# chaitjo/efficient-gnns

Measured on NVIDIA H100. Metric: edges aggregated/s (fwd+bwd), 3-layer GCN student + logit-KD, ARXIV-shape, higher is better.
Workload: dtype f32

## Files before the change

efficient-gnns_b200/csrc/gemm_wgrad_tf32x3.cu:

```cuda
#include "common.cuh"
#include "tc_common.cuh"

namespace b200gnn {
namespace wgrad {
using namespace tc;

constexpr int BKN = 32;
constexpr int TM = 128, TN = 128;
constexpr int THREADS = 384;
constexpr int STAGES = 5;
constexpr int X_BOX = 8;
constexpr int RAW_BYTES = BKN * (TM + TN) * 4;
constexpr int OP_BYTES = 128 * BKN * 4;
constexpr int T_BYTES = 2 * OP_BYTES;
constexpr int SS_BYTES = TM / 2 * 16;
constexpr int SMEM_BYTES = STAGES * RAW_BYTES + 2 * T_BYTES + 256 + SS_BYTES + 1024;
constexpr int MAX_RANGES = 132;
constexpr int64_t MAX_PARTIAL_FLOATS = (int64_t)MAX_RANGES * 256 * 256;
constexpr int MAX_KIN = 2048, MAX_NOUT = 512;
static_assert(SMEM_BYTES <= 232448, "shared memory");

struct Params {
  float* partial;
  int32_t Nn, Kin, Kpad, Nout, Npad, num_kb;
  int32_t n_tn, n_ranges;
  const float* act_scale;
  const float* act_shift;
  const uint32_t* act_bits;
  int32_t act_words;
  float inv_keep;
  const float* act_slope;
  int32_t act_ld;
};

template <bool ACT, bool PRELU = false>
__global__ void __launch_bounds__(THREADS, 1)
wgrad_tf32x3_kernel(const __grid_constant__ CUtensorMap tmX, const __grid_constant__ CUtensorMap tmG, const Params p) {
  extern __shared__ uint8_t smem_raw[];
  uint8_t* smem = reinterpret_cast<uint8_t*>((reinterpret_cast<uintptr_t>(smem_raw) + 1023) & ~(uintptr_t)1023);
  uint8_t* tbuf = smem + STAGES * RAW_BYTES;
  uint64_t* full = reinterpret_cast<uint64_t*>(tbuf + 2 * T_BYTES);
  uint64_t* empty = full + STAGES;
  float4* act_ss = reinterpret_cast<float4*>(tbuf + 2 * T_BYTES + 256);

  const int tiles = (p.Kpad / TM) * p.n_tn;
  const int tile = (int)blockIdx.x % tiles, range = (int)blockIdx.x / tiles;
  const int mt = tile / p.n_tn, nt = tile % p.n_tn;
  const int kb0 = (int)((int64_t)p.num_kb * range / p.n_ranges);
  const int kb1 = (int)((int64_t)p.num_kb * (range + 1) / p.n_ranges);

  const int warp = threadIdx.x >> 5, lane = threadIdx.x & 31;
  if (threadIdx.x == 0) {
    for (int s = 0; s < STAGES; ++s) { mbar_init(&full[s], 1); mbar_init(&empty[s], 256); }
    asm volatile("fence.mbarrier_init.release.cluster;" ::: "memory");
  }
  __syncthreads();

  if (warp < 4) {
    regs_dec<40>();
    if (threadIdx.x == 0) {
      int s = 0; uint32_t ph = 0;
      for (int kb = kb0; kb < kb1; ++kb) {
        mbar_wait(&empty[s], ph ^ 1);
        uint8_t* st = smem + s * RAW_BYTES;
        mbar_expect_tx(&full[s], RAW_BYTES);
        for (int j = 0; j < TM / X_BOX; ++j)
          tma_load_2d(&tmX, &full[s], st + j * BKN * X_BOX * 4, mt * TM + j * X_BOX, kb * BKN);
        tma_load_2d(&tmG, &full[s], st + BKN * TM * 4, nt * TN, kb * BKN);
        if (++s == STAGES) { s = 0; ph ^= 1; }
      }
    }
    return;
  }
  regs_inc<232>();

  const int cw = (warp >> 2) - 1;
  const int ct = threadIdx.x - 128;
  const uint32_t xfrag = (8 * cw + 2 * (warp & 3)) * (BKN * X_BOX * 4) + (lane & 3) * (X_BOX * 4) + (lane >> 2) * 4;
  const int pair = cw * 32 + (warp & 3) * 8 + (lane >> 2);
  const int c0 = mt * TM + cw * 64 + (warp & 3) * 16 + (lane >> 2);
  uint32_t wnext = 0u;
  const int bits_ld = PRELU ? p.act_ld : p.act_words;
  auto act_word = [&](int kb) {
    const int node = kb * BKN + lane;
    return node < p.Nn && (c0 >> 5) < p.act_words ? __ldg(p.act_bits + (size_t)node * bits_ld + (c0 >> 5)) : 0u;
  };
  const float slope = PRELU ? __ldg(p.act_slope) : 0.f;
  if (PRELU && kb0 < kb1) wnext = act_word(kb0);
  if (ACT) {
    if (ct < TM / 2) {
      const int c = mt * TM + (ct >> 3) * 16 + (ct & 7);
      float4 v = make_float4(0.f, 0.f, 0.f, 0.f);
      if (c < p.Kin) { v.x = __ldg(p.act_scale + c); v.y = __ldg(p.act_shift + c); }
      if (c + 8 < p.Kin) { v.z = __ldg(p.act_scale + c + 8); v.w = __ldg(p.act_shift + c + 8); }
      act_ss[ct] = v;
    }
    if (kb0 < kb1) wnext = act_word(kb0);
    named_sync(1, 256);
  }
  float acc[64], sum[64];
#pragma unroll
  for (int i = 0; i < 64; ++i) sum[i] = acc[i] = 0.f;
  uint32_t xh0[BKN / 8][4], xl0[BKN / 8][4], xh1[BKN / 8][4], xl1[BKN / 8][4];
  int s = 0; uint32_t ph = 0;
  auto block = [&](int i, uint32_t (&h)[BKN / 8][4], uint32_t (&l)[BKN / 8][4]) {
    uint32_t wcur = 0u;
    if (ACT || PRELU) {
      wcur = wnext;
      if (kb0 + i + 1 < kb1) wnext = act_word(kb0 + i + 1);
    }
    mbar_wait(&full[s], ph);
    float4 ss = make_float4(0.f, 0.f, 0.f, 0.f);
    int l4 = lane & 3;
    if (ACT) {
      ss = act_ss[pair];
      asm volatile("" : "+r"(l4));
    }
    if (PRELU) asm volatile("" : "+r"(l4));
    const uint32_t sraw = smem_u32(smem + s * RAW_BYTES);
    const float* rg = reinterpret_cast<const float*>(smem + s * RAW_BYTES + BKN * TM * 4);
    uint8_t* T = tbuf + (i & 1) * T_BYTES;
#pragma unroll
    for (int u = 0; u < 4; ++u) {
      const int idx = u * 256 + ct;
      const int r = idx & 127, c = idx >> 7;
      const float* src = rg + (4 * c) * 128 + r;
      const uint4 v = make_uint4(__float_as_uint(src[0]), __float_as_uint(src[128]), __float_as_uint(src[256]),
                                 __float_as_uint(src[384]));
      uint4 hv, lv;
      split4(v, hv, lv);
      *reinterpret_cast<uint4*>(T + swz128(r, c)) = hv;
      *reinterpret_cast<uint4*>(T + OP_BYTES + swz128(r, c)) = lv;
    }
#pragma unroll
    for (int k = 0; k < BKN / 8; ++k)
#pragma unroll
      for (int j = 0; j < 4; ++j) {
        uint32_t v = lds32(sraw + xfrag + (j & 1) * (BKN * X_BOX * 4) + (8 * k + 4 * (j >> 1)) * (X_BOX * 4));
        if (ACT) {
          const uint32_t w = __shfl_sync(0xffffffffu, wcur, 8 * k + l4 + 4 * (j >> 1));
          const float y = fmaxf(fmaf(__uint_as_float(v), (j & 1) ? ss.z : ss.x, (j & 1) ? ss.w : ss.y), 0.f) * p.inv_keep;
          v = (w >> ((c0 & 31) + 8 * (j & 1))) & 1u ? __float_as_uint(y) : 0u;
        }
        if (PRELU) {
          const uint32_t w = __shfl_sync(0xffffffffu, wcur, 8 * k + l4 + 4 * (j >> 1));
          const float z = __uint_as_float(v);
          const float y = (z > 0.f ? z : slope * z) * p.inv_keep;
          v = (w >> ((c0 & 31) + 8 * (j & 1))) & 1u ? __float_as_uint(y) : 0u;
        }
        split1(v, h[k][j], l[k][j]);
      }
    asm volatile("fence.proxy.async.shared::cta;" ::: "memory");
    mbar_arrive(&empty[s]);
    if (i > 0) {
      wgmma_wait<0>();
      acc_fence(acc);
#pragma unroll
      for (int j = 0; j < 64; ++j) sum[j] += acc[j];
    }
    named_sync(1, 256);
    reg_fence(h); reg_fence(l);
    wgmma_fence();
    const uint32_t sa = smem_u32(T);
#pragma unroll
    for (int k = 0; k < BKN / 8; ++k) {
      const uint32_t koff = k * 32;
      wgmma_tf32_n128_rs(acc, l[k], make_desc_k128(sa + koff), k != 0);
      wgmma_tf32_n128_rs(acc, h[k], make_desc_k128(sa + OP_BYTES + koff), 1);
    }
#pragma unroll
    for (int k = 0; k < BKN / 8; ++k) wgmma_tf32_n128_rs(acc, h[k], make_desc_k128(sa + k * 32), 1);
    wgmma_commit();
    if (++s == STAGES) { s = 0; ph ^= 1; }
  };
  for (int i = 0; i < kb1 - kb0; i += 2) {
    block(i, xh0, xl0);
    if (i + 1 < kb1 - kb0) block(i + 1, xh1, xl1);
  }
  if (kb1 > kb0) {
    wgmma_wait<0>();
    acc_fence(acc);
#pragma unroll
    for (int j = 0; j < 64; ++j) sum[j] += acc[j];
  }
  float* out = p.partial + (size_t)range * p.Kpad * p.Npad;
  const int row0 = mt * TM + cw * 64 + (warp & 3) * 16 + (lane >> 2);
#pragma unroll
  for (int j = 0; j < 16; ++j) {
    const int col = nt * TN + 8 * j + 2 * (lane & 3);
    if (col < p.Npad) {
      *reinterpret_cast<float2*>(out + (size_t)row0 * p.Npad + col) = make_float2(sum[4 * j], sum[4 * j + 1]);
      *reinterpret_cast<float2*>(out + (size_t)(row0 + 8) * p.Npad + col) = make_float2(sum[4 * j + 2], sum[4 * j + 3]);
    }
  }
}

constexpr int RED_VECS = 32, RED_GROUPS = 8;
__global__ void __launch_bounds__(RED_VECS * RED_GROUPS) wgrad_reduce_kernel(const float4* __restrict__ partial, int n_part,
                                                                             int Kin, int Kpad, int Nout, int Npad,
                                                                             float* __restrict__ out) {
  __shared__ float4 sh[RED_GROUPS][RED_VECS];
  const int64_t n_vec = (int64_t)Kpad * Npad / 4;
  const int v = threadIdx.x % RED_VECS, g = threadIdx.x / RED_VECS;
  const int64_t i = (int64_t)blockIdx.x * RED_VECS + v;
  float4 acc = make_float4(0.f, 0.f, 0.f, 0.f);
  if (i < n_vec)
    for (int c = g; c < n_part; c += RED_GROUPS) {
      const float4 x = __ldcs(partial + (size_t)c * n_vec + i);
      acc.x += x.x; acc.y += x.y; acc.z += x.z; acc.w += x.w;
    }
  sh[g][v] = acc;
  __syncthreads();
  if (g != 0 || i >= n_vec) return;
  const int row = (int)(i / (Npad / 4)), c4 = (int)(i % (Npad / 4)) * 4;
  if (c4 >= Nout || row >= Kin) return;
#pragma unroll
  for (int j = 1; j < RED_GROUPS; ++j) {
    const float4 x = sh[j][v];
    acc.x += x.x; acc.y += x.y; acc.z += x.z; acc.w += x.w;
  }
  *reinterpret_cast<float4*>(out + (size_t)row * Nout + c4) = acc;
}

static bool make_map_rows(CUtensorMap* m, const float* base, int64_t rows, int64_t width, int64_t ld, int box_cols) {
  EncodeTiledFn fn = encode_fn();
  if (!fn) return false;
  cuuint64_t dims[2] = {(cuuint64_t)width, (cuuint64_t)rows};
  cuuint64_t strides[1] = {(cuuint64_t)ld * 4};
  cuuint32_t box[2] = {(cuuint32_t)box_cols, (cuuint32_t)BKN};
  cuuint32_t estr[2] = {1, 1};
  return fn(m, CU_TENSOR_MAP_DATA_TYPE_FLOAT32, 2, const_cast<float*>(base), dims, strides, box, estr,
            CU_TENSOR_MAP_INTERLEAVE_NONE, CU_TENSOR_MAP_SWIZZLE_NONE, CU_TENSOR_MAP_L2_PROMOTION_L2_256B,
            CU_TENSOR_MAP_FLOAT_OOB_FILL_NONE) == CUDA_SUCCESS;
}

static int64_t pad_k(int64_t Kin) { return (Kin + TM - 1) / TM * TM; }
static int64_t pad_n(int64_t Nout) { return (Nout + 31) / 32 * 32; }
static int range_cap(int64_t Kin, int64_t Nout) {
  const int64_t c = MAX_PARTIAL_FLOATS / (pad_k(Kin) * pad_n(Nout));
  return (int)(c > MAX_RANGES ? MAX_RANGES : (c < 1 ? 1 : c));
}

}
}

using namespace b200gnn;

extern "C" int64_t b200gnn_wgrad_workspace_floats(int64_t Kin, int64_t Nout) {
  if (Kin <= 0 || Nout <= 0) return B200GNN_ERR_BAD_ARG;
  if (Kin > wgrad::MAX_KIN || Nout > wgrad::MAX_NOUT) return B200GNN_ERR_UNSUPPORTED;
  return wgrad::range_cap(Kin, Nout) * wgrad::pad_k(Kin) * wgrad::pad_n(Nout);
}

template <bool ACT, bool PRELU = false>
static int wgrad_launch(const float* X, int64_t ldx, const float* G, int64_t ldg, float* dW, int64_t Nn, int64_t Kin, int64_t Nout,
                        float* workspace, const wgrad::Params& act, void* stream) {
  if (!X || !G || !dW || !workspace || Nn <= 0 || Kin <= 0 || Nout <= 0 || ldx < Kin || ldg < Nout || Nn >= INT32_MAX)
    return B200GNN_ERR_BAD_ARG;
  if (Kin % 4 || Kin > wgrad::MAX_KIN || Nout % 4 || Nout > wgrad::MAX_NOUT || ldx % 4 || ldg % 4 || !aligned_to(X, 16) || !aligned_to(G, 16) ||
      !aligned_to(dW, 16) || !aligned_to(workspace, 16))
    return B200GNN_ERR_UNSUPPORTED;
  CUtensorMap tX, tG;
  if (!wgrad::make_map_rows(&tX, X, Nn, Kin, ldx, wgrad::X_BOX) || !wgrad::make_map_rows(&tG, G, Nn, Nout, ldg, wgrad::TN))
    return B200GNN_ERR_UNSUPPORTED;
  int dev = 0, sms = 132;
  cudaGetDevice(&dev);
  static bool attr_set[64] = {};
  if (dev >= 0 && dev < 64 && !attr_set[dev]) {
    cudaError_t e = cudaFuncSetAttribute(wgrad::wgrad_tf32x3_kernel<ACT, PRELU>, cudaFuncAttributeMaxDynamicSharedMemorySize,
                                         wgrad::SMEM_BYTES);
    if (e != cudaSuccess) { set_cuda_error(e); return B200GNN_ERR_CUDA; }
    attr_set[dev] = true;
  }
  cudaDeviceGetAttribute(&sms, cudaDevAttrMultiProcessorCount, dev);
  cudaStream_t st = (cudaStream_t)stream;
  wgrad::Params p = act;
  p.partial = workspace; p.Nn = (int32_t)Nn; p.Kin = (int32_t)Kin; p.Nout = (int32_t)Nout;
  p.Kpad = (int32_t)wgrad::pad_k(Kin);
  p.Npad = (int32_t)wgrad::pad_n(Nout);
  p.num_kb = (int32_t)((Nn + wgrad::BKN - 1) / wgrad::BKN);
  p.n_tn = (p.Npad + wgrad::TN - 1) / wgrad::TN;
  const int tiles = (int)(p.Kpad / wgrad::TM) * p.n_tn;
  int ranges = sms / tiles;
  const int cap = wgrad::range_cap(Kin, Nout);
  if (ranges > cap) ranges = cap;
  if (ranges > p.num_kb) ranges = p.num_kb;
  if (ranges < 1) ranges = 1;
  p.n_ranges = ranges;
  int rc;
  wgrad::wgrad_tf32x3_kernel<ACT, PRELU><<<tiles * ranges, wgrad::THREADS, wgrad::SMEM_BYTES, st>>>(tX, tG, p);
  if ((rc = check_launch())) return rc;
  const int64_t n_vec = (int64_t)p.Kpad * p.Npad / 4;
  wgrad::wgrad_reduce_kernel<<<(int)((n_vec + wgrad::RED_VECS - 1) / wgrad::RED_VECS), wgrad::RED_VECS * wgrad::RED_GROUPS, 0, st>>>(
      reinterpret_cast<const float4*>(workspace), ranges, (int)Kin, p.Kpad, (int)Nout, p.Npad, dW);
  return check_launch();
}

extern "C" int b200gnn_gemm_wgrad_tf32x3_f32(const float* X, int64_t ldx, const float* G, int64_t ldg, float* dW,
                                             int64_t Nn, int64_t Kin, int64_t Nout, float* workspace, void* stream) {
  return wgrad_launch<false>(X, ldx, G, ldg, dW, Nn, Kin, Nout, workspace, wgrad::Params{}, stream);
}

extern "C" int b200gnn_gemm_wgrad_tf32x3_act_f32(const float* Y, int64_t ldx, const float* G, int64_t ldg, float* dW,
                                                 int64_t Nn, int64_t Kin, int64_t Nout, const float* scale, const float* shift,
                                                 const uint32_t* bits, float p_drop, float* workspace, void* stream) {
  if (!scale || !shift || !bits || p_drop < 0.f || p_drop >= 1.f) return B200GNN_ERR_BAD_ARG;
  wgrad::Params act{};
  act.act_scale = scale; act.act_shift = shift; act.act_bits = bits; act.act_words = (int32_t)((Kin + 31) / 32);
  act.inv_keep = p_drop > 0.f ? 1.f / (1.f - p_drop) : 1.f;
  return wgrad_launch<true>(Y, ldx, G, ldg, dW, Nn, Kin, Nout, workspace, act, stream);
}

extern "C" int b200gnn_gemm_wgrad_tf32x3_prelu_f32(const float* Z, int64_t ldz, const float* G, int64_t ldg, float* dW,
                                                   int64_t Nn, int64_t Kin, int64_t Nout, const float* slope,
                                                   const uint32_t* bits, int64_t ldbits, float p_drop, float* workspace,
                                                   void* stream) {
  if (!slope || !bits || ldbits < (Kin + 31) / 32 || ldbits >= INT32_MAX || p_drop < 0.f || p_drop >= 1.f)
    return B200GNN_ERR_BAD_ARG;
  wgrad::Params act{};
  act.act_slope = slope; act.act_bits = bits; act.act_words = (int32_t)((Kin + 31) / 32); act.act_ld = (int32_t)ldbits;
  act.inv_keep = p_drop > 0.f ? 1.f / (1.f - p_drop) : 1.f;
  return wgrad_launch<false, true>(Z, ldz, G, ldg, dW, Nn, Kin, Nout, workspace, act, stream);
}
```

efficient-gnns_b200/csrc/tc_common.cuh:

```cuda
#pragma once
#include <cuda.h>
#include <cuda_runtime.h>
#include <stdint.h>

namespace b200gnn {
namespace tc {

constexpr uint32_t TF32_MASK = 0xFFFFE000u;

__device__ __forceinline__ uint32_t smem_u32(const void* p) { return (uint32_t)__cvta_generic_to_shared(p); }

__device__ __forceinline__ void mbar_init(uint64_t* bar, uint32_t count) {
  asm volatile("mbarrier.init.shared::cta.b64 [%0], %1;" ::"r"(smem_u32(bar)), "r"(count));
}
__device__ __forceinline__ void mbar_arrive(uint64_t* bar) {
  asm volatile("mbarrier.arrive.shared::cta.b64 _, [%0];" ::"r"(smem_u32(bar)) : "memory");
}
__device__ __forceinline__ void mbar_expect_tx(uint64_t* bar, uint32_t bytes) {
  asm volatile("mbarrier.arrive.expect_tx.shared::cta.b64 _, [%0], %1;" ::"r"(smem_u32(bar)), "r"(bytes) : "memory");
}
__device__ __forceinline__ bool mbar_try_wait(uint64_t* bar, uint32_t parity) {
  uint32_t ok;
  asm volatile(
      "{\n\t"
      ".reg .pred p;\n\t"
      "mbarrier.try_wait.parity.shared::cta.b64 p, [%1], %2;\n\t"
      "selp.u32 %0, 1, 0, p;\n\t"
      "}"
      : "=r"(ok)
      : "r"(smem_u32(bar)), "r"(parity)
      : "memory");
  return ok != 0;
}
__device__ __forceinline__ void mbar_wait(uint64_t* bar, uint32_t parity) {
  while (!mbar_try_wait(bar, parity)) {}
}

__device__ __forceinline__ void tma_load_2d(const CUtensorMap* tmap, uint64_t* bar, void* dst, int c0, int c1) {
  asm volatile(
      "cp.async.bulk.tensor.2d.shared::cluster.global.mbarrier::complete_tx::bytes [%0], [%1, {%3, %4}], [%2];"
      ::"r"(smem_u32(dst)), "l"(reinterpret_cast<uint64_t>(tmap)), "r"(smem_u32(bar)), "r"(c0), "r"(c1)
      : "memory");
}

__device__ __forceinline__ uint32_t lds32(uint32_t saddr) {
  uint32_t v;
  asm volatile("ld.shared.b32 %0, [%1];" : "=r"(v) : "r"(saddr) : "memory");
  return v;
}

__device__ __forceinline__ void named_sync(uint32_t id, uint32_t count) {
  asm volatile("bar.sync %0, %1;" ::"r"(id), "r"(count) : "memory");
}

template <uint32_t N> __device__ __forceinline__ void regs_dec() { asm volatile("setmaxnreg.dec.sync.aligned.u32 %0;" ::"n"(N)); }
template <uint32_t N> __device__ __forceinline__ void regs_inc() { asm volatile("setmaxnreg.inc.sync.aligned.u32 %0;" ::"n"(N)); }

__device__ __forceinline__ uint64_t make_desc_k128(uint32_t saddr) {
  uint64_t d = 0;
  d |= (uint64_t)((saddr & 0x3FFFF) >> 4);
  d |= (uint64_t)1 << 16;
  d |= (uint64_t)(1024 >> 4) << 32;
  d |= (uint64_t)1 << 62;
  return d;
}
__device__ __forceinline__ uint32_t swz128(int r, int c) { return (uint32_t)(r * 128 + ((c ^ (r & 7)) << 4)); }

__device__ __forceinline__ void wgmma_fence() { asm volatile("wgmma.fence.sync.aligned;" ::: "memory"); }
__device__ __forceinline__ void wgmma_commit() { asm volatile("wgmma.commit_group.sync.aligned;" ::: "memory"); }
template <int N> __device__ __forceinline__ void wgmma_wait() { asm volatile("wgmma.wait_group.sync.aligned %0;" ::"n"(N) : "memory"); }
template <int R> __device__ __forceinline__ void acc_fence(float (&d)[R]) {
#pragma unroll
  for (int i = 0; i < R; ++i) asm volatile("" : "+f"(d[i])::"memory");
}

__device__ __forceinline__ void wgmma_tf32_n128_rs(float (&d)[64], const uint32_t (&a)[4], uint64_t db, uint32_t scale_d) {
  asm volatile(
      "{\n\t.reg .pred p;\n\tsetp.ne.b32 p, %69, 0;\n\t"
      "wgmma.mma_async.sync.aligned.m64n128k8.f32.tf32.tf32 {%0,%1,%2,%3,%4,%5,%6,%7,%8,%9,%10,%11,%12,%13,%14,%15,%16,%17,%18,%19,%20,%21,%22,%23,%24,%25,%26,%27,%28,%29,%30,%31,%32,%33,%34,%35,%36,%37,%38,%39,%40,%41,%42,%43,%44,%45,%46,%47,%48,%49,%50,%51,%52,%53,%54,%55,%56,%57,%58,%59,%60,%61,%62,%63}, {%64,%65,%66,%67}, %68, p, 1, 1;\n\t}"
      : "+f"(d[0]), "+f"(d[1]), "+f"(d[2]), "+f"(d[3]), "+f"(d[4]), "+f"(d[5]), "+f"(d[6]), "+f"(d[7]), "+f"(d[8]), "+f"(d[9]), "+f"(d[10]), "+f"(d[11]), "+f"(d[12]), "+f"(d[13]), "+f"(d[14]), "+f"(d[15]), "+f"(d[16]), "+f"(d[17]), "+f"(d[18]), "+f"(d[19]), "+f"(d[20]), "+f"(d[21]), "+f"(d[22]), "+f"(d[23]), "+f"(d[24]), "+f"(d[25]), "+f"(d[26]), "+f"(d[27]), "+f"(d[28]), "+f"(d[29]), "+f"(d[30]), "+f"(d[31]), "+f"(d[32]), "+f"(d[33]), "+f"(d[34]), "+f"(d[35]), "+f"(d[36]), "+f"(d[37]), "+f"(d[38]), "+f"(d[39]), "+f"(d[40]), "+f"(d[41]), "+f"(d[42]), "+f"(d[43]), "+f"(d[44]), "+f"(d[45]), "+f"(d[46]), "+f"(d[47]), "+f"(d[48]), "+f"(d[49]), "+f"(d[50]), "+f"(d[51]), "+f"(d[52]), "+f"(d[53]), "+f"(d[54]), "+f"(d[55]), "+f"(d[56]), "+f"(d[57]), "+f"(d[58]), "+f"(d[59]), "+f"(d[60]), "+f"(d[61]), "+f"(d[62]), "+f"(d[63])
      : "r"(a[0]), "r"(a[1]), "r"(a[2]), "r"(a[3]), "l"(db), "r"(scale_d));
}
__device__ __forceinline__ void wgmma_tf32_n48_rs(float (&d)[24], const uint32_t (&a)[4], uint64_t db, uint32_t scale_d) {
  asm volatile(
      "{\n\t.reg .pred p;\n\tsetp.ne.b32 p, %29, 0;\n\t"
      "wgmma.mma_async.sync.aligned.m64n48k8.f32.tf32.tf32 {%0,%1,%2,%3,%4,%5,%6,%7,%8,%9,%10,%11,%12,%13,%14,%15,%16,%17,%18,%19,%20,%21,%22,%23}, {%24,%25,%26,%27}, %28, p, 1, 1;\n\t}"
      : "+f"(d[0]), "+f"(d[1]), "+f"(d[2]), "+f"(d[3]), "+f"(d[4]), "+f"(d[5]), "+f"(d[6]), "+f"(d[7]), "+f"(d[8]), "+f"(d[9]), "+f"(d[10]), "+f"(d[11]), "+f"(d[12]), "+f"(d[13]), "+f"(d[14]), "+f"(d[15]), "+f"(d[16]), "+f"(d[17]), "+f"(d[18]), "+f"(d[19]), "+f"(d[20]), "+f"(d[21]), "+f"(d[22]), "+f"(d[23])
      : "r"(a[0]), "r"(a[1]), "r"(a[2]), "r"(a[3]), "l"(db), "r"(scale_d));
}
template <int K> __device__ __forceinline__ void reg_fence(uint32_t (&r)[K][4]) {
#pragma unroll
  for (int k = 0; k < K; ++k)
#pragma unroll
    for (int i = 0; i < 4; ++i) asm volatile("" : "+r"(r[k][i])::"memory");
}

__device__ __forceinline__ uint32_t rna_tf32(float x) { return (__float_as_uint(x) + 0x1000u) & TF32_MASK; }
__device__ __forceinline__ void split1(uint32_t v, uint32_t& h, uint32_t& l) {
  h = rna_tf32(__uint_as_float(v));
  l = rna_tf32(__uint_as_float(v) - __uint_as_float(h));
}
__device__ __forceinline__ void split4(const uint4& v, uint4& h, uint4& l) {
  split1(v.x, h.x, l.x); split1(v.y, h.y, l.y); split1(v.z, h.z, l.z); split1(v.w, h.w, l.w);
}

typedef CUresult (*EncodeTiledFn)(CUtensorMap*, CUtensorMapDataType, cuuint32_t, void*, const cuuint64_t*, const cuuint64_t*,
                                  const cuuint32_t*, const cuuint32_t*, CUtensorMapInterleave, CUtensorMapSwizzle,
                                  CUtensorMapL2promotion, CUtensorMapFloatOOBfill);

inline EncodeTiledFn encode_fn() {
  static EncodeTiledFn fn = nullptr;
  if (!fn) {
    void* p = nullptr;
    cudaDriverEntryPointQueryResult q;
    if (cudaGetDriverEntryPoint("cuTensorMapEncodeTiled", &p, cudaEnableDefault, &q) == cudaSuccess &&
        q == cudaDriverEntryPointSuccess)
      fn = reinterpret_cast<EncodeTiledFn>(p);
  }
  return fn;
}

}
}
```

Before: 3.978 billion.

## Pipeline wgrad WGMMA with split accumulators and add narrow-N tile variant

Restructures the TF32x3 weight-gradient kernel so the 128-wide tile issues two n64 WGMMA groups into separate accumulators, and promotion into the fp32 sum overlaps with in-flight MMAs through wait<1>. The split of the next block is moved after the MMA issue, with triple-buffered transposed operands, so splitting overlaps tensor-core work. A TN=48 specialization with more pipeline stages is added for outputs of 48 columns or fewer, such as the logit layer, to avoid wasted N padding. The cost is more template variants and more complex wait ordering, and the 128 path drops from 5 to 4 stages.

```diff
diff --git a/efficient-gnns_b200/csrc/gemm_wgrad_tf32x3.cu b/efficient-gnns_b200/csrc/gemm_wgrad_tf32x3.cu
--- a/efficient-gnns_b200/csrc/gemm_wgrad_tf32x3.cu
+++ b/efficient-gnns_b200/csrc/gemm_wgrad_tf32x3.cu
@@ -6,19 +6,25 @@
 using namespace tc;
 
 constexpr int BKN = 32;
-constexpr int TM = 128, TN = 128;
+constexpr int TM = 128;
 constexpr int THREADS = 384;
-constexpr int STAGES = 5;
 constexpr int X_BOX = 8;
-constexpr int RAW_BYTES = BKN * (TM + TN) * 4;
-constexpr int OP_BYTES = 128 * BKN * 4;
-constexpr int T_BYTES = 2 * OP_BYTES;
 constexpr int SS_BYTES = TM / 2 * 16;
-constexpr int SMEM_BYTES = STAGES * RAW_BYTES + 2 * T_BYTES + 256 + SS_BYTES + 1024;
+constexpr int NT = 3;
+constexpr int U = 4;
+template <int TN> struct Tile {
+  static constexpr int RAW_BYTES = BKN * (TM + TN) * 4;
+  static constexpr int OP_BYTES = TN * BKN * 4;
+  static constexpr int T_BYTES = 2 * OP_BYTES;
+  static constexpr int STAGES = TN == 128 ? 4 : 8;
+  static constexpr int SMEM_BYTES = STAGES * RAW_BYTES + NT * T_BYTES + 256 + SS_BYTES + 1024;
+  static constexpr int ACC = TN == 128 ? 32 : 24;
+};
+static_assert(Tile<128>::SMEM_BYTES <= 232448, "shared memory");
+static_assert(Tile<48>::SMEM_BYTES <= 232448, "shared memory");
 constexpr int MAX_RANGES = 132;
 constexpr int64_t MAX_PARTIAL_FLOATS = (int64_t)MAX_RANGES * 256 * 256;
 constexpr int MAX_KIN = 2048, MAX_NOUT = 512;
-static_assert(SMEM_BYTES <= 232448, "shared memory");
 
 struct Params {
   float* partial;
@@ -33,15 +39,35 @@
   int32_t act_ld;
 };
 
-template <bool ACT, bool PRELU = false>
+__device__ __forceinline__ void mma(float (&d)[32], const uint32_t (&a)[4], uint64_t b, uint32_t s) { wgmma_tf32_n64_rs(d, a, b, s); }
+__device__ __forceinline__ void mma(float (&d)[24], const uint32_t (&a)[4], uint64_t b, uint32_t s) { wgmma_tf32_n48_rs(d, a, b, s); }
+
+template <int TN, int R>
+__device__ __forceinline__ void block_mma(float (&d)[R], const uint32_t (&h)[BKN / 8][4], const uint32_t (&l)[BKN / 8][4],
+                                          uint32_t sb) {
+  wgmma_fence();
+#pragma unroll
+  for (int k = 0; k < BKN / 8; ++k) {
+    const uint32_t koff = k * 32;
+    mma(d, l[k], make_desc_k128(sb + koff), k != 0);
+    mma(d, h[k], make_desc_k128(sb + Tile<TN>::OP_BYTES + koff), 1);
+  }
+#pragma unroll
+  for (int k = 0; k < BKN / 8; ++k) mma(d, h[k], make_desc_k128(sb + k * 32), 1);
+  wgmma_commit();
+}
+
+template <int TN, bool ACT, bool PRELU = false>
 __global__ void __launch_bounds__(THREADS, 1)
 wgrad_tf32x3_kernel(const __grid_constant__ CUtensorMap tmX, const __grid_constant__ CUtensorMap tmG, const Params p) {
+  using C = Tile<TN>;
+  constexpr int STAGES = C::STAGES, RAW_BYTES = C::RAW_BYTES, T_BYTES = C::T_BYTES, R = C::ACC;
   extern __shared__ uint8_t smem_raw[];
   uint8_t* smem = reinterpret_cast<uint8_t*>((reinterpret_cast<uintptr_t>(smem_raw) + 1023) & ~(uintptr_t)1023);
   uint8_t* tbuf = smem + STAGES * RAW_BYTES;
-  uint64_t* full = reinterpret_cast<uint64_t*>(tbuf + 2 * T_BYTES);
+  uint64_t* full = reinterpret_cast<uint64_t*>(tbuf + NT * T_BYTES);
   uint64_t* empty = full + STAGES;
-  float4* act_ss = reinterpret_cast<float4*>(tbuf + 2 * T_BYTES + 256);
+  float4* act_ss = reinterpret_cast<float4*>(tbuf + NT * T_BYTES + 256);
 
   const int tiles = (p.Kpad / TM) * p.n_tn;
   const int tile = (int)blockIdx.x % tiles, range = (int)blockIdx.x / tiles;
@@ -98,18 +124,26 @@
     if (kb0 < kb1) wnext = act_word(kb0);
     named_sync(1, 256);
   }
-  float acc[64], sum[64];
-#pragma unroll
-  for (int i = 0; i < 64; ++i) sum[i] = acc[i] = 0.f;
+  float acc0[R], acc1[R], sum[TN / 2];
+#pragma unroll
+  for (int i = 0; i < R; ++i) acc0[i] = acc1[i] = 0.f;
+#pragma unroll
+  for (int i = 0; i < TN / 2; ++i) sum[i] = 0.f;
+  auto promote = [&](float (&d)[R], int off) {
+    acc_fence(d);
+#pragma unroll
+    for (int j = 0; j < R; ++j) sum[off + j] += d[j];
+  };
   uint32_t xh0[BKN / 8][4], xl0[BKN / 8][4], xh1[BKN / 8][4], xl1[BKN / 8][4];
-  int s = 0; uint32_t ph = 0;
-  auto block = [&](int i, uint32_t (&h)[BKN / 8][4], uint32_t (&l)[BKN / 8][4]) {
+  const int n = kb1 - kb0;
+  auto split = [&](int i, uint32_t (&h)[BKN / 8][4], uint32_t (&l)[BKN / 8][4]) {
     uint32_t wcur = 0u;
     if (ACT || PRELU) {
       wcur = wnext;
-      if (kb0 + i + 1 < kb1) wnext = act_word(kb0 + i + 1);
-    }
-    mbar_wait(&full[s], ph);
+      if (i + 1 < n) wnext = act_word(kb0 + i + 1);
+    }
+    const int s = i % STAGES;
+    mbar_wait(&full[s], (uint32_t)(i / STAGES) & 1u);
     float4 ss = make_float4(0.f, 0.f, 0.f, 0.f);
     int l4 = lane & 3;
     if (ACT) {
@@ -119,18 +153,21 @@
     if (PRELU) asm volatile("" : "+r"(l4));
     const uint32_t sraw = smem_u32(smem + s * RAW_BYTES);
     const float* rg = reinterpret_cast<const float*>(smem + s * RAW_BYTES + BKN * TM * 4);
-    uint8_t* T = tbuf + (i & 1) * T_BYTES;
-#pragma unroll
-    for (int u = 0; u < 4; ++u) {
+    uint8_t* T = tbuf + (i % NT) * T_BYTES;
+    constexpr int ITEMS = TN * BKN / 4;
+#pragma unroll
+    for (int u = 0; u < (ITEMS + 255) / 256; ++u) {
       const int idx = u * 256 + ct;
-      const int r = idx & 127, c = idx >> 7;
-      const float* src = rg + (4 * c) * 128 + r;
-      const uint4 v = make_uint4(__float_as_uint(src[0]), __float_as_uint(src[128]), __float_as_uint(src[256]),
-                                 __float_as_uint(src[384]));
-      uint4 hv, lv;
-      split4(v, hv, lv);
-      *reinterpret_cast<uint4*>(T + swz128(r, c)) = hv;
-      *reinterpret_cast<uint4*>(T + OP_BYTES + swz128(r, c)) = lv;
+      if (ITEMS % 256 == 0 || idx < ITEMS) {
+        const int r = idx % TN, c = idx / TN;
+        const float* src = rg + (4 * c) * TN + r;
+        const uint4 v = make_uint4(__float_as_uint(src[0]), __float_as_uint(src[TN]), __float_as_uint(src[2 * TN]),
+                                   __float_as_uint(src[3 * TN]));
+        uint4 hv, lv;
+        split4(v, hv, lv);
+        *reinterpret_cast<uint4*>(T + swz128(r, c)) = hv;
+        *reinterpret_cast<uint4*>(T + C::OP_BYTES + swz128(r, c)) = lv;
+      }
     }
 #pragma unroll
     for (int k = 0; k < BKN / 8; ++k)
@@ -152,41 +189,50 @@
       }
     asm volatile("fence.proxy.async.shared::cta;" ::: "memory");
     mbar_arrive(&empty[s]);
-    if (i > 0) {
-      wgmma_wait<0>();
-      acc_fence(acc);
-#pragma unroll
-      for (int j = 0; j < 64; ++j) sum[j] += acc[j];
-    }
+  };
+  auto step = [&](int i, const int u, const bool first) {
+    uint32_t(&h)[BKN / 8][4] = (u & 1) ? xh1 : xh0;
+    uint32_t(&l)[BKN / 8][4] = (u & 1) ? xl1 : xl0;
     named_sync(1, 256);
     reg_fence(h); reg_fence(l);
-    wgmma_fence();
-    const uint32_t sa = smem_u32(T);
-#pragma unroll
-    for (int k = 0; k < BKN / 8; ++k) {
-      const uint32_t koff = k * 32;
-      wgmma_tf32_n128_rs(acc, l[k], make_desc_k128(sa + koff), k != 0);
-      wgmma_tf32_n128_rs(acc, h[k], make_desc_k128(sa + OP_BYTES + koff), 1);
-    }
-#pragma unroll
-    for (int k = 0; k < BKN / 8; ++k) wgmma_tf32_n128_rs(acc, h[k], make_desc_k128(sa + k * 32), 1);
-    wgmma_commit();
-    if (++s == STAGES) { s = 0; ph ^= 1; }
-  };
-  for (int i = 0; i < kb1 - kb0; i += 2) {
-    block(i, xh0, xl0);
-    if (i + 1 < kb1 - kb0) block(i + 1, xh1, xl1);
-  }
-  if (kb1 > kb0) {
+    const uint32_t sa = smem_u32(tbuf + (i % NT) * T_BYTES);
+    if constexpr (TN == 128) {
+      if (!first) { wgmma_wait<1>(); promote(acc0, 0); }
+      block_mma<TN>(acc0, h, l, sa);
+      if (!first) { wgmma_wait<1>(); promote(acc1, R); }
+      block_mma<TN>(acc1, h, l, sa + 64 * 128);
+    } else {
+      block_mma<TN>((u & 1) ? acc1 : acc0, h, l, sa);
+      if (!first) { wgmma_wait<1>(); promote((u & 1) ? acc0 : acc1, 0); }
+    }
+    if (i + 1 < n) split(i + 1, (u & 1) ? xh0 : xh1, (u & 1) ? xl0 : xl1);
+  };
+  auto drain = [&](const int u) {
     wgmma_wait<0>();
-    acc_fence(acc);
-#pragma unroll
-    for (int j = 0; j < 64; ++j) sum[j] += acc[j];
-  }
+    if constexpr (TN == 128) {
+      promote(acc0, 0);
+      promote(acc1, R);
+    } else {
+      promote((u & 1) ? acc1 : acc0, 0);
+    }
+  };
+  if (n > 0) split(0, xh0, xl0);
+  int i = 0;
+  for (; i + U <= n; i += U) {
+#pragma unroll
+    for (int u = 0; u < U; ++u) step(i + u, u, u == 0);
+    drain(U - 1);
+  }
+#pragma unroll
+  for (int u = 0; u < U - 1; ++u)
+    if (i + u < n) {
+      step(i + u, u, true);
+      drain(u);
+    }
   float* out = p.partial + (size_t)range * p.Kpad * p.Npad;
   const int row0 = mt * TM + cw * 64 + (warp & 3) * 16 + (lane >> 2);
 #pragma unroll
-  for (int j = 0; j < 16; ++j) {
+  for (int j = 0; j < TN / 8; ++j) {
     const int col = nt * TN + 8 * j + 2 * (lane & 3);
     if (col < p.Npad) {
       *reinterpret_cast<float2*>(out + (size_t)row0 * p.Npad + col) = make_float2(sum[4 * j], sum[4 * j + 1]);
@@ -252,6 +298,35 @@
   return wgrad::range_cap(Kin, Nout) * wgrad::pad_k(Kin) * wgrad::pad_n(Nout);
 }
 
+template <int TN, bool ACT, bool PRELU>
+static int wgrad_launch_tn(const CUtensorMap& tX, const float* G, int64_t ldg, wgrad::Params p, float* dW, int dev, int sms,
+                           cudaStream_t st) {
+  CUtensorMap tG;
+  if (!wgrad::make_map_rows(&tG, G, p.Nn, p.Nout, ldg, TN)) return B200GNN_ERR_UNSUPPORTED;
+  static bool attr_set[64] = {};
+  if (dev >= 0 && dev < 64 && !attr_set[dev]) {
+    cudaError_t e = cudaFuncSetAttribute(wgrad::wgrad_tf32x3_kernel<TN, ACT, PRELU>, cudaFuncAttributeMaxDynamicSharedMemorySize,
+                                         wgrad::Tile<TN>::SMEM_BYTES);
+    if (e != cudaSuccess) { set_cuda_error(e); return B200GNN_ERR_CUDA; }
+    attr_set[dev] = true;
+  }
+  p.n_tn = TN == 48 ? 1 : (p.Npad + TN - 1) / TN;
+  const int tiles = (int)(p.Kpad / wgrad::TM) * p.n_tn;
+  int ranges = sms / tiles;
+  const int cap = wgrad::range_cap(p.Kin, p.Nout);
+  if (ranges > cap) ranges = cap;
+  if (ranges > p.num_kb) ranges = p.num_kb;
+  if (ranges < 1) ranges = 1;
+  p.n_ranges = ranges;
+  int rc;
+  wgrad::wgrad_tf32x3_kernel<TN, ACT, PRELU><<<tiles * ranges, wgrad::THREADS, wgrad::Tile<TN>::SMEM_BYTES, st>>>(tX, tG, p);
+  if ((rc = check_launch())) return rc;
+  const int64_t n_vec = (int64_t)p.Kpad * p.Npad / 4;
+  wgrad::wgrad_reduce_kernel<<<(int)((n_vec + wgrad::RED_VECS - 1) / wgrad::RED_VECS), wgrad::RED_VECS * wgrad::RED_GROUPS, 0, st>>>(
+      reinterpret_cast<const float4*>(p.partial), ranges, p.Kin, p.Kpad, p.Nout, p.Npad, dW);
+  return check_launch();
+}
+
 template <bool ACT, bool PRELU = false>
 static int wgrad_launch(const float* X, int64_t ldx, const float* G, int64_t ldg, float* dW, int64_t Nn, int64_t Kin, int64_t Nout,
                         float* workspace, const wgrad::Params& act, void* stream) {
@@ -260,40 +335,19 @@
   if (Kin % 4 || Kin > wgrad::MAX_KIN || Nout % 4 || Nout > wgrad::MAX_NOUT || ldx % 4 || ldg % 4 || !aligned_to(X, 16) || !aligned_to(G, 16) ||
       !aligned_to(dW, 16) || !aligned_to(workspace, 16))
     return B200GNN_ERR_UNSUPPORTED;
-  CUtensorMap tX, tG;
-  if (!wgrad::make_map_rows(&tX, X, Nn, Kin, ldx, wgrad::X_BOX) || !wgrad::make_map_rows(&tG, G, Nn, Nout, ldg, wgrad::TN))
-    return B200GNN_ERR_UNSUPPORTED;
+  CUtensorMap tX;
+  if (!wgrad::make_map_rows(&tX, X, Nn, Kin, ldx, wgrad::X_BOX)) return B200GNN_ERR_UNSUPPORTED;
   int dev = 0, sms = 132;
   cudaGetDevice(&dev);
-  static bool attr_set[64] = {};
-  if (dev >= 0 && dev < 64 && !attr_set[dev]) {
-    cudaError_t e = cudaFuncSetAttribute(wgrad::wgrad_tf32x3_kernel<ACT, PRELU>, cudaFuncAttributeMaxDynamicSharedMemorySize,
-                                         wgrad::SMEM_BYTES);
-    if (e != cudaSuccess) { set_cuda_error(e); return B200GNN_ERR_CUDA; }
-    attr_set[dev] = true;
-  }
   cudaDeviceGetAttribute(&sms, cudaDevAttrMultiProcessorCount, dev);
-  cudaStream_t st = (cudaStream_t)stream;
   wgrad::Params p = act;
   p.partial = workspace; p.Nn = (int32_t)Nn; p.Kin = (int32_t)Kin; p.Nout = (int32_t)Nout;
   p.Kpad = (int32_t)wgrad::pad_k(Kin);
   p.Npad = (int32_t)wgrad::pad_n(Nout);
   p.num_kb = (int32_t)((Nn + wgrad::BKN - 1) / wgrad::BKN);
-  p.n_tn = (p.Npad + wgrad::TN - 1) / wgrad::TN;
-  const int tiles = (int)(p.Kpad / wgrad::TM) * p.n_tn;
-  int ranges = sms / tiles;
-  const int cap = wgrad::range_cap(Kin, Nout);
-  if (ranges > cap) ranges = cap;
-  if (ranges > p.num_kb) ranges = p.num_kb;
-  if (ranges < 1) ranges = 1;
-  p.n_ranges = ranges;
-  int rc;
-  wgrad::wgrad_tf32x3_kernel<ACT, PRELU><<<tiles * ranges, wgrad::THREADS, wgrad::SMEM_BYTES, st>>>(tX, tG, p);
-  if ((rc = check_launch())) return rc;
-  const int64_t n_vec = (int64_t)p.Kpad * p.Npad / 4;
-  wgrad::wgrad_reduce_kernel<<<(int)((n_vec + wgrad::RED_VECS - 1) / wgrad::RED_VECS), wgrad::RED_VECS * wgrad::RED_GROUPS, 0, st>>>(
-      reinterpret_cast<const float4*>(workspace), ranges, (int)Kin, p.Kpad, (int)Nout, p.Npad, dW);
-  return check_launch();
+  cudaStream_t st = (cudaStream_t)stream;
+  return Nout <= 48 ? wgrad_launch_tn<48, ACT, PRELU>(tX, G, ldg, p, dW, dev, sms, st)
+                    : wgrad_launch_tn<128, ACT, PRELU>(tX, G, ldg, p, dW, dev, sms, st);
 }
 
 extern "C" int b200gnn_gemm_wgrad_tf32x3_f32(const float* X, int64_t ldx, const float* G, int64_t ldg, float* dW,
diff --git a/efficient-gnns_b200/csrc/tc_common.cuh b/efficient-gnns_b200/csrc/tc_common.cuh
--- a/efficient-gnns_b200/csrc/tc_common.cuh
+++ b/efficient-gnns_b200/csrc/tc_common.cuh
@@ -81,6 +81,13 @@
       : "+f"(d[0]), "+f"(d[1]), "+f"(d[2]), "+f"(d[3]), "+f"(d[4]), "+f"(d[5]), "+f"(d[6]), "+f"(d[7]), "+f"(d[8]), "+f"(d[9]), "+f"(d[10]), "+f"(d[11]), "+f"(d[12]), "+f"(d[13]), "+f"(d[14]), "+f"(d[15]), "+f"(d[16]), "+f"(d[17]), "+f"(d[18]), "+f"(d[19]), "+f"(d[20]), "+f"(d[21]), "+f"(d[22]), "+f"(d[23]), "+f"(d[24]), "+f"(d[25]), "+f"(d[26]), "+f"(d[27]), "+f"(d[28]), "+f"(d[29]), "+f"(d[30]), "+f"(d[31]), "+f"(d[32]), "+f"(d[33]), "+f"(d[34]), "+f"(d[35]), "+f"(d[36]), "+f"(d[37]), "+f"(d[38]), "+f"(d[39]), "+f"(d[40]), "+f"(d[41]), "+f"(d[42]), "+f"(d[43]), "+f"(d[44]), "+f"(d[45]), "+f"(d[46]), "+f"(d[47]), "+f"(d[48]), "+f"(d[49]), "+f"(d[50]), "+f"(d[51]), "+f"(d[52]), "+f"(d[53]), "+f"(d[54]), "+f"(d[55]), "+f"(d[56]), "+f"(d[57]), "+f"(d[58]), "+f"(d[59]), "+f"(d[60]), "+f"(d[61]), "+f"(d[62]), "+f"(d[63])
       : "r"(a[0]), "r"(a[1]), "r"(a[2]), "r"(a[3]), "l"(db), "r"(scale_d));
 }
+__device__ __forceinline__ void wgmma_tf32_n64_rs(float (&d)[32], const uint32_t (&a)[4], uint64_t db, uint32_t scale_d) {
+  asm volatile(
+      "{\n\t.reg .pred p;\n\tsetp.ne.b32 p, %37, 0;\n\t"
+      "wgmma.mma_async.sync.aligned.m64n64k8.f32.tf32.tf32 {%0,%1,%2,%3,%4,%5,%6,%7,%8,%9,%10,%11,%12,%13,%14,%15,%16,%17,%18,%19,%20,%21,%22,%23,%24,%25,%26,%27,%28,%29,%30,%31}, {%32,%33,%34,%35}, %36, p, 1, 1;\n\t}"
+      : "+f"(d[0]), "+f"(d[1]), "+f"(d[2]), "+f"(d[3]), "+f"(d[4]), "+f"(d[5]), "+f"(d[6]), "+f"(d[7]), "+f"(d[8]), "+f"(d[9]), "+f"(d[10]), "+f"(d[11]), "+f"(d[12]), "+f"(d[13]), "+f"(d[14]), "+f"(d[15]), "+f"(d[16]), "+f"(d[17]), "+f"(d[18]), "+f"(d[19]), "+f"(d[20]), "+f"(d[21]), "+f"(d[22]), "+f"(d[23]), "+f"(d[24]), "+f"(d[25]), "+f"(d[26]), "+f"(d[27]), "+f"(d[28]), "+f"(d[29]), "+f"(d[30]), "+f"(d[31])
+      : "r"(a[0]), "r"(a[1]), "r"(a[2]), "r"(a[3]), "l"(db), "r"(scale_d));
+}
 __device__ __forceinline__ void wgmma_tf32_n48_rs(float (&d)[24], const uint32_t (&a)[4], uint64_t db, uint32_t scale_d) {
   asm volatile(
       "{\n\t.reg .pred p;\n\tsetp.ne.b32 p, %29, 0;\n\t"
```

Result: no change. 4.011 billion (median of 6 runs) (+0.8%).
